# Tariq-Abuhashim/semantic-slam

Measured on AMD Instinct MI355X. Metric: Mvoxels/sec integrated, 512³ grid @ 640×480 depth; achieved HBM GB/s %peak, higher is better.
Workload: dtype f32

## Files before the change

### include/tsdf_hip_diag.h

```cpp
#ifndef TSDF_HIP_DIAG_H
#define TSDF_HIP_DIAG_H

#include "tsdf_hip.h"

#ifdef __cplusplus
extern "C" {
#endif


int tsdf_integrate_sequence_timed(tsdf_volume *vol, const float *depth_dev, const float *cam2world,
                                  int32_t n_frames, float *elapsed_ms);

int tsdf_integrate_frames_timed(tsdf_volume *vol, const float *const *depth_dev, const uint8_t *const *masks_dev,
                                const float *cam2world, int32_t n_frames, float *elapsed_ms);


int tsdf_probe_graph_replay(tsdf_volume *vol, const float *depth_dev, const float *cam2world, int32_t n_frames,
                            int32_t iters, float *ms_launches, float *ms_graph);

int tsdf_probe_stream(tsdf_volume *vol, int32_t non_temporal, int32_t n_iters, float *elapsed_ms);


int tsdf_selftest_fastdiv(int32_t device, uint64_t seed, uint64_t n_samples, float fx, float cx,
                          uint64_t *mismatches, float first_bad[4]);

int tsdf_selftest_fastdiv_band(int32_t device, uint64_t seed, uint64_t n_samples, uint64_t *mismatches,
                               float first_bad[4]);

int tsdf_selftest_round(int32_t device, uint64_t *mismatches, float first_bad[4]);

int tsdf_selftest_tile_tables(int32_t device, const float *depth_dev, const uint8_t *mask_dev, int32_t im_height,
                              int32_t im_width, float max_depth, uint64_t *mismatches);


int32_t tsdf_frames_per_launch(const tsdf_volume *vol);
int tsdf_shortcut_stats(tsdf_volume *vol, int32_t enable, uint64_t counts_out[3]);
int tsdf_brick_list_stats(tsdf_volume *vol, uint64_t counts_out[4]);
int tsdf_classification_info(tsdf_volume *vol, double info_out[2]);

int tsdf_summary_stats(tsdf_volume *vol, uint64_t out[3]);
int tsdf_summary_words(tsdf_volume *vol, uint32_t *out_host, int64_t capacity, int64_t *count);

int tsdf_store_stats(tsdf_volume *vol, int64_t out[9]);

int tsdf_last_cam2base(const tsdf_volume *vol, float out[16]);


int tsdf_set_kernel_variant(tsdf_volume *vol, int32_t variant);

int tsdf_set_brick_shape(tsdf_volume *vol, int32_t quads, int32_t rows, int32_t slices);
int tsdf_brick_shape(const tsdf_volume *vol, int32_t shape_out[3]);
int tsdf_default_brick_shape(const tsdf_config *cfg, int32_t shape_out[3]);

#ifdef __cplusplus
}
#endif
#endif
```

### semantic_slam_amd/capi.py

```python
import ctypes as C
import os

import numpy as np

_PKG = os.path.dirname(os.path.abspath(__file__))
LIB_PATH = os.environ.get("TSDF_HIP_LIB") or os.path.join(_PKG, "libtsdf_hip.so")

ABI_SYMBOLS = [
    "tsdf_config_default", "tsdf_create", "tsdf_destroy", "tsdf_reset", "tsdf_integrate",
    "tsdf_integrate_u16", "tsdf_convert_depth_u16", "tsdf_set_deferral",
    "tsdf_integrate_device", "tsdf_integrate_cam2base", "tsdf_integrate_masked_device",
    "tsdf_integrate_frames_device",
    "tsdf_sync", "tsdf_download", "tsdf_copy_slices", "tsdf_upload", "tsdf_refresh_summary", "tsdf_device_ptrs", "tsdf_slab_voxels", "tsdf_frames_per_launch", "tsdf_shortcut_stats", "tsdf_brick_list_stats", "tsdf_classification_info", "tsdf_store_stats", "tsdf_summary_stats", "tsdf_summary_words",
    "tsdf_get_config", "tsdf_last_cam2base", "tsdf_set_stream", "tsdf_get_stream",
    "tsdf_count_surface", "tsdf_extract_surface", "tsdf_extract_crossings", "tsdf_extract_mesh", "tsdf_save_mesh_ply", "tsdf_save_mesh_welded_ply", "tsdf_save_ply", "tsdf_save_bin", "tsdf_load_bin", "tsdf_save_state", "tsdf_load_state",
    "tsdf_integrate_sequence_timed", "tsdf_integrate_frames_timed", "tsdf_probe_graph_replay", "tsdf_probe_stream", "tsdf_selftest_fastdiv", "tsdf_selftest_fastdiv_band", "tsdf_selftest_round", "tsdf_selftest_tile_tables", "tsdf_set_kernel_variant", "tsdf_set_brick_shape", "tsdf_brick_shape", "tsdf_default_brick_shape", "tsdf_last_error",
    "tsdf_version", "tsdf_multiply_matrix", "tsdf_invert_matrix",
    "tsdf_labels_enable", "tsdf_compose_labels", "tsdf_integrate_labels_device", "tsdf_integrate_frames_labels_device",
    "tsdf_download_labels",
    "tsdf_colour_enable", "tsdf_integrate_colour_device", "tsdf_integrate_rgbd", "tsdf_download_colour",
    "tsdf_raycast_params_default", "tsdf_raycast_device", "tsdf_raycast", "tsdf_batch_raycast_device",
    "tsdf_track_params_default", "tsdf_track", "tsdf_track_system",
    "tsdf_photo_params_default", "tsdf_track_rgbd", "tsdf_track_rgbd_system", "tsdf_render_intensity",
    "tsdf_batch_track", "tsdf_batch_track_system", "tsdf_track_member_systems",
    "tsdf_fuse_params_default", "tsdf_fuse_volume",
    "tsdf_align_params_default", "tsdf_fuse_pose_default", "tsdf_align_volume", "tsdf_align_system", "tsdf_fuse_volume_at",
    "tsdf_fuse_volume_carry", "tsdf_upload_labels", "tsdf_upload_colour",
    "tsdf_extent_params_default", "tsdf_volume_extent", "tsdf_batch_extents", "tsdf_group_extent", "tsdf_extent_combine",
    "tsdf_extent_metric", "tsdf_extent_regrid",
    "tsdf_associate_params_default", "tsdf_associate_count", "tsdf_associate_assign", "tsdf_batch_associate",
    "tsdf_segment_params_default", "tsdf_segmenter_create", "tsdf_segmenter_destroy", "tsdf_segmenter_set_stream",
    "tsdf_segment_depth_device", "tsdf_segment_refine_masks_device", "tsdf_segment_frame",
    "tsdf_object_origin", "tsdf_batch_create", "tsdf_batch_destroy", "tsdf_batch_size", "tsdf_batch_volume",
    "tsdf_batch_integrate_device", "tsdf_batch_sync",
    "tsdf_group_create", "tsdf_group_destroy", "tsdf_group_size", "tsdf_group_voxels", "tsdf_group_volume",
    "tsdf_group_integrate", "tsdf_group_integrate_frames", "tsdf_group_set_deferral", "tsdf_group_sync", "tsdf_group_reset", "tsdf_group_download",
    "tsdf_group_extract_surface", "tsdf_group_extract_crossings", "tsdf_group_extract_mesh",
    "tsdf_group_save_ply", "tsdf_group_save_mesh_ply", "tsdf_group_save_bin",
]
DIAG_SYMBOLS = [
    "tsdf_integrate_sequence_timed", "tsdf_integrate_frames_timed",
    "tsdf_probe_graph_replay", "tsdf_probe_stream",
    "tsdf_selftest_fastdiv", "tsdf_selftest_fastdiv_band", "tsdf_selftest_round", "tsdf_selftest_tile_tables",
    "tsdf_shortcut_stats", "tsdf_brick_list_stats", "tsdf_classification_info", "tsdf_store_stats", "tsdf_summary_stats", "tsdf_summary_words", "tsdf_frames_per_launch", "tsdf_last_cam2base",
    "tsdf_set_kernel_variant", "tsdf_set_brick_shape", "tsdf_brick_shape", "tsdf_default_brick_shape",
]


class TsdfError(RuntimeError):
    pass


SHIPPED_VARIANTS = (0, 1, 3, 7, 8)


def experiments_build():
    return b"+experiments" in load().tsdf_version()


def variants(*wanted):
# ... 147 lines not shown
    L.tsdf_integrate_masked_device.argtypes = [vp, vp, vp, vp]
    L.tsdf_integrate_frames_device.argtypes = [vp, vp, vp, vp, C.c_int32]
    L.tsdf_sync.argtypes = [vp]
    L.tsdf_download.argtypes = [vp, vp, vp]
    L.tsdf_upload.argtypes = [vp, vp, vp]
    L.tsdf_copy_slices.argtypes = [vp, C.c_int32, C.c_int32, vp, vp]
    L.tsdf_refresh_summary.argtypes = [vp]
    L.tsdf_device_ptrs.argtypes = [vp, C.POINTER(vp), C.POINTER(vp)]
    L.tsdf_slab_voxels.argtypes = [vp]
    L.tsdf_slab_voxels.restype = C.c_int64
    L.tsdf_frames_per_launch.argtypes = [vp]
    L.tsdf_frames_per_launch.restype = C.c_int32
    L.tsdf_shortcut_stats.argtypes = [vp, C.c_int32, vp]
    L.tsdf_classification_info.argtypes = [vp, vp]
    L.tsdf_brick_list_stats.argtypes = [vp, vp]
    if hasattr(L, "tsdf_store_stats"):
        L.tsdf_store_stats.argtypes = [vp, i64p]
    if hasattr(L, "tsdf_summary_stats"):
        L.tsdf_summary_stats.argtypes = [vp, vp]
    if hasattr(L, "tsdf_summary_words"):
        L.tsdf_summary_words.argtypes = [vp, vp, C.c_int64, i64p]
    L.tsdf_get_config.argtypes = [vp, C.POINTER(TsdfConfig)]
    L.tsdf_last_cam2base.argtypes = [vp, vp]
    L.tsdf_set_stream.argtypes = [vp, vp]
    L.tsdf_get_stream.argtypes = [vp, C.POINTER(vp)]
    L.tsdf_count_surface.argtypes = [vp, C.c_float, i64p]
    L.tsdf_extract_surface.argtypes = [vp, C.c_float, vp, C.c_int64, i64p]
    L.tsdf_extract_crossings.argtypes = [vp, vp, vp, C.c_float, vp, C.c_int64, i64p]
    L.tsdf_extract_mesh.argtypes = [vp, vp, vp, C.c_float, vp, C.c_int64, i64p]
    L.tsdf_save_mesh_ply.argtypes = [vp, C.c_char_p, C.c_float]
# ... 401 lines not shown
    def shortcut_stats(self, enable=True):
        out = (C.c_uint64 * 3)()
        check(self.lib.tsdf_shortcut_stats(self._h, 1 if enable else 0, out), "tsdf_shortcut_stats")
        return tuple(int(x) for x in out)

    def brick_list_stats(self):
        out = (C.c_uint64 * 4)()
        check(self.lib.tsdf_brick_list_stats(self._h, out), "tsdf_brick_list_stats")
        return tuple(int(x) for x in out)

    def classification_info(self):
        out = (C.c_double * 2)()
        check(self.lib.tsdf_classification_info(self._h, out), "tsdf_classification_info")
        return float(out[0]), int(out[1])

    def store_stats(self):
        out = (C.c_int64 * 9)()
        check(self.lib.tsdf_store_stats(self._h, out), "tsdf_store_stats")
        return {name: tuple(int(x) for x in out[3 * k:3 * k + 3]) for k, name in enumerate(("frames", "masks", "tables"))}

    def summary_stats(self):
        out = (C.c_uint64 * 3)()
        check(self.lib.tsdf_summary_stats(self._h, out), "tsdf_summary_stats")
        return tuple(int(x) for x in out)

    def summary_words(self):
        n = C.c_int64(0)
        check(self.lib.tsdf_summary_words(self._h, None, 0, C.byref(n)), "tsdf_summary_words")
        out = np.zeros(int(n.value), np.uint32)
        if out.size:
# ... 607 lines not shown
```

### semantic_slam_amd/csrc/host_derive.h

```cpp
#pragma once
#include <algorithm>
#include <cmath>
#include <cstddef>
#include <cstdint>

#include "tsdf_hip.h"

namespace tsdf_host {

inline bool brick_shape_ok(const tsdf_config &c, int q, int r, int s)
{
    return c.dim_x % 4 == 0 && q >= 1 && r >= 1 && s >= 1 && q * r * s <= 64 && (c.dim_x / 4) % q == 0 &&
           (long long)s * c.dim_x * c.dim_y < (1ll << 30);
}

inline void choose_brick_default(const tsdf_config &c, int &bq, int &br, int &bs)
{
    bq = 0; br = 0; bs = 1;
    if (c.dim_x % 4 != 0) return;
    const int quads = c.dim_x / 4;
    const int nz = c.z_end - c.z_begin;
    double best = 1e300;
    for (int q = 1; q <= 64 && q <= quads; ++q) {
        if (quads % q) continue;
// ... 132 lines not shown
constexpr int64_t kClassifyMinVoxels = 48000000;
inline bool classify_one_frame(Classify mode, int64_t launch_voxels)
{
    if (mode == Classify::Never) return false;
    return mode == Classify::Always || launch_voxels >= kClassifyMinVoxels;
}

constexpr double kMinClaimFraction = 0.10;
constexpr int kProbeEvery = 8;
inline bool classify_fused(Classify mode, bool claims_known, double claim_fraction, int launches_unclassified)
{
    if (mode != Classify::Adaptive) return mode == Classify::Always;
    return !claims_known || claim_fraction >= kMinClaimFraction || launches_unclassified >= kProbeEvery - 1;
}

constexpr int64_t kWindowBytes = 512ll << 20;

struct SweepWindow { int cache_lo, cache_hi; };

inline SweepWindow sweep_window(int nz, int dim_x, int dim_y, int64_t window_bytes, bool reverse)
{
    const int64_t slice_bytes = 8 * (int64_t)dim_x * dim_y;
    const int w = (int)std::min<int64_t>(nz, window_bytes / slice_bytes);
    return reverse ? SweepWindow{0, w} : SweepWindow{nz - w, nz};
}

inline bool batch_defers(int members, int64_t total_voxels) { return 2 * (int64_t)members < 10 + total_voxels / 1000000; }

constexpr int64_t kBatchMinVoxelsPerMember = 2000000;
inline bool batch_classifies(Classify mode, int members, int64_t launch_voxels)
// ... 45 lines not shown
```

### semantic_slam_amd/csrc/launch_geometry.h

```cpp
#pragma once
#include <algorithm>
#include <cmath>
#include <cstddef>
#include <cstdint>

#include "host_derive.h"

namespace tsdf_host {

enum class ConfigLimit { Ok, GridDims, SlabRange, ImageSize, VoxelAndTrunc, LaunchLimits, SliceVoxels };

constexpr int kMaxDimY = 65535 * 4, kMaxSlices = 65535;
constexpr int64_t kMaxSliceVoxels = ((int64_t)1 << 31) - 1024, kMaxImagePixels = (int64_t)1 << 30;

inline ConfigLimit config_limits_ok(const tsdf_config &c)
{
    if (c.dim_x <= 0 || c.dim_y <= 0 || c.dim_z <= 0) return ConfigLimit::GridDims;
    if (c.z_begin < 0 || c.z_end < c.z_begin || c.z_end > c.dim_z) return ConfigLimit::SlabRange;
    if (c.im_height <= 0 || c.im_width <= 0 || (int64_t)c.im_height * c.im_width > kMaxImagePixels) return ConfigLimit::ImageSize;
    if (!(c.voxel_size > 0.0f) || !(c.trunc_margin > 0.0f)) return ConfigLimit::VoxelAndTrunc;
    if (c.dim_y > kMaxDimY || (c.z_end - c.z_begin) > kMaxSlices) return ConfigLimit::LaunchLimits;
    if ((int64_t)c.dim_x * c.dim_y > kMaxSliceVoxels) return ConfigLimit::SliceVoxels;
    return ConfigLimit::Ok;
}
// ... 57 lines not shown
inline Grid3 grid_quad_rows(const SlabGeometry &g, int rows_per_wg)
{
    return {(unsigned)ceil_div(g.xgroups(4), 64), (unsigned)ceil_div(g.dim_y, rows_per_wg), (unsigned)g.nz};
}
inline Grid3 grid_flat(const SlabGeometry &g) { return {(unsigned)ceil_div(g.chunks_per_slice, 4), 1u, (unsigned)g.nz}; }
inline Grid3 grid_recompute_flags(const SlabGeometry &g) { return grid_flat(g); }

inline int brick_blocks(const SlabGeometry &g) { return ceil_div(g.brick_groups * g.bricks_per_group, 4); }
struct BrickGrid { Grid3 grid; size_t class_elems; };
inline BrickGrid brick_grid(int blocks, int slice_groups)
{
    return {{(unsigned)blocks, 1u, (unsigned)slice_groups}, (size_t)blocks * (size_t)slice_groups * 4};
}
inline BrickGrid brick_grid(const SlabGeometry &g) { return brick_grid(brick_blocks(g), g.nz_groups); }

constexpr size_t kStridePassBlocks = 256 * 8;
inline Grid3 grid_summary_words(const SlabGeometry &g) { return {(unsigned)std::min((g.n_flags + 255) / 256, kStridePassBlocks), 1u, 1u}; }
inline Grid3 grid_fill(const SlabGeometry &g)
{
    return {(unsigned)std::max<size_t>(std::min(((size_t)g.n_vox / 4 + 255) / 256, kStridePassBlocks), 1), 1u, 1u};
}

inline Grid3 grid_tile_strips(int tiles_w, int tiles_h, int tile, int frames)
{
    const int strips = ceil_div(tiles_w, 64 / tile) * tiles_h;
    return {(unsigned)ceil_div(strips, 4), (unsigned)frames, 1u};
}

constexpr int kListBuckets = 64;
constexpr int kSuperBX = 4, kSuperBY = 2, kSuperBZ = 1;
// ... 102 lines not shown
```

### semantic_slam_amd/csrc/tsdf_capi.hip

```cpp
#include "../../include/tsdf_hip.h"
#include "../../include/tsdf_hip_diag.h"

#include <hip/hip_runtime.h>

#include <algorithm>
#include <cmath>
#include <cstdarg>
#include <cstdio>
#include <cstdlib>
#include <cstring>
#include <new>
#include <string>
#include <vector>

#include "pose_math.h"
#include "host_derive.h"
#include "launch_geometry.h"
#include "host_copy.h"
#include "hip_owned.h"
#include "frame_store.h"
#include "tsdf_kernels.hip.h"
#include "tsdf_multiframe.hip.h"
#include "tsdf_labels.hip.h"
#include "tsdf_colour.hip.h"
// ... 102 lines not shown
    DevPtr<unsigned long long> d_claims;
    HostPtr<unsigned long long> h_claims;
    Event claims_done;
    Stream pre_stream, rb_stream;
    int rb_parity = -1;
    Event pre_done[2], list_free[2], seq_ready;
    int list_parity = 0;
    bool list_used[2] = {false, false};
    bool pipeline_ok = false;
    bool claims_pending = false, claims_known = false;
    double claims_total = 0.0;
    double claim_fraction = 0.0;
    int launches_unclassified = 0;
    DevBuf<char> d_scratch;
    DevBuf<uint8_t> d_wg_class;
    DevBuf<char> d_list;
    DevBuf<char> d_track;
    HostPtr<tsdfk::TrackState> h_track;
    DevBuf<char> d_photo;
    HostBuf<char> h_photo;
    DevPtr<unsigned long long> d_fuse;
    HostPtr<unsigned long long> h_fuse;
    Event fuse_src_ready, fuse_done;
    DevPtr<char> d_align;
    HostPtr<tsdfk::TrackState> h_align;
    Event align_src_ready, align_done;
    DevPtr<unsigned long long> d_extent;
    HostPtr<unsigned long long> h_extent;
};

// ... 336 lines not shown
{
    int64_t window = tsdf_host::kWindowBytes;
    bool forward_only = false;
#ifdef TSDF_EXPERIMENTS
    if (const char *e = std::getenv("TSDF_MALL_WINDOW_MB")) window = (int64_t)std::atoi(e) << 20;
    forward_only = std::getenv("TSDF_SWEEP_FORWARD") && std::atoi(std::getenv("TSDF_SWEEP_FORWARD")) != 0;
    p.head_plain_loads = std::getenv("TSDF_HEAD_PLAIN_LOADS") && std::atoi(std::getenv("TSDF_HEAD_PLAIN_LOADS")) != 0;
#endif
    p.sweep_reverse = forward_only ? 0 : v->sweep_parity;
    v->sweep_parity ^= 1;
    const tsdf_host::SweepWindow w = tsdf_host::sweep_window(p.nz, p.dim_x, p.dim_y, window, p.sweep_reverse != 0);
    p.cache_lo = w.cache_lo;
    p.cache_hi = w.cache_hi;
}

int launch_integrate(tsdf_volume *v, const float *depth_dev, const uint8_t *mask_dev,
                     const float *c2b)
{
    const tsdf_host::SlabGeometry &geo = v->geo;
    if (geo.nz == 0) return TSDF_OK;
    std::memcpy(v->last_cam2base, c2b, sizeof v->last_cam2base);
#ifdef TSDF_EXPERIMENTS
    if (geo.quad_rows && (v->variant == 2 || (v->variant >= 16 && !mask_dev) ||
                          (v->variant == 11 && mask_dev && !geo.flat && tiles_fit(geo.tiles_w, geo.tiles_h))))
        return launch_integrate_experiment(v, depth_dev, mask_dev, c2b);
#endif
    const tsdf_host::OneFrame one = tsdf_host::one_frame(geo, variant_of(v->variant), mask_dev != nullptr, tiles_fit(geo.tiles_w, geo.tiles_h));
    if (one.kernel == tsdf_host::OneFrameKernel::Scalar) {
        int rc = summary_before(v, one.keeps);
        if (rc) return rc;
// ... 1 lines not shown
        const dim3 block(64, 4, 1), grid = to_dim3(tsdf_host::grid_scalar_rows(geo));
        if (mask_dev) hipLaunchKernelGGL((tsdfk::integrate_scalar<true>), grid, block, 0, v->stream, p);
        else hipLaunchKernelGGL((tsdfk::integrate_scalar<false>), grid, block, 0, v->stream, p);
        HIP_TRY(hipGetLastError());
        return TSDF_OK;
    }
    if (geo.flat) {
        return launch_multi(v, &depth_dev, mask_dev ? &mask_dev : nullptr, c2b, 1);
    }
    tsdfk::IntegrateParams p = make_params(v, depth_dev, mask_dev, c2b, 4);
    if (one.kernel == tsdf_host::OneFrameKernel::MaskedBricks) return launch_masked_bricks(v, p);
    int rc = summary_before(v, one.keeps);
    if (rc) return rc;
    const dim3 block(64, 4, 1), grid = to_dim3(tsdf_host::grid_quad_rows(geo, 8));
    set_sweep(v, p);
    if (mask_dev) hipLaunchKernelGGL((tsdfk::integrate_tile<2, true>), grid, block, 0, v->stream, p);
    else hipLaunchKernelGGL((tsdfk::integrate_tile<2, false>), grid, block, 0, v->stream, p);
    HIP_TRY(hipGetLastError());
    return TSDF_OK;
}

void compose_cam2base(const tsdf_volume *v, const float *cam2world, float *c2b)
{
    tsdf_host::multiply_matrix(v->base2world_inv, cam2world, c2b);
}

int launch_multi(tsdf_volume *v, const float *const *depth_dev, const uint8_t *const *masks_dev,
                 const float *c2b, int n, const uint16_t *const *label_ims, const float *const *score_ims, hipEvent_t inputs_ready)
{
    const tsdf_config &c = v->cfg;
    const tsdf_host::SlabGeometry &geo = v->geo;
    if (geo.nz == 0 || n == 0) return TSDF_OK;
    {
        int rc = summary_before(v, tsdf_host::Keeps::Bits);
// ... 936 lines not shown
```

### semantic_slam_amd/csrc/tsdf_diag.hip.h

```cpp
#pragma once

namespace {

template <typename Queue>
int time_on_stream(tsdf_volume *v, const char *who, float *elapsed_ms, Queue &&queue)
{
    Event e0, e1;
    HIP_TRY(event_create(e0, hipEventDefault));
    HIP_TRY(event_create(e1, hipEventDefault));
    HIP_TRY(hipEventRecord(e0, v->stream));
    const int rc = queue();
    hipError_t er = hipEventRecord(e1, v->stream);
    hipError_t es = hipEventSynchronize(e1);
    float ms = 0.f;
    hipError_t et = hipEventElapsedTime(&ms, e0, e1);
    if (rc) return rc;
    if (er != hipSuccess || es != hipSuccess || et != hipSuccess)
        return fail(TSDF_ERR_HIP, "%s: event timing failed", who);
    *elapsed_ms = ms;
    return TSDF_OK;
}

int frames_timed(tsdf_volume *v, const float *const *depth_dev, const uint8_t *const *masks_dev,
                 const float *cam2world, int32_t n_frames, float *elapsed_ms, const char *who)
// ... 257 lines not shown
{
    if (!v) return fail(TSDF_ERR_INVALID, "tsdf_shortcut_stats: NULL handle");
    int rc = bind_device(v);
    if (rc) return rc;
    HIP_TRY(hipStreamSynchronize(v->stream));
    if (counts_out) {
        unsigned int h[3] = {0, 0, 0};
        if (v->d_shortcut_stats) HIP_TRY(hipMemcpy(h, v->d_shortcut_stats, sizeof h, hipMemcpyDeviceToHost));
        for (int i = 0; i < 3; ++i) counts_out[i] = h[i];
    }
    if (enable && !v->d_shortcut_stats) HIP_TRY(dev_alloc(v->d_shortcut_stats, 8 * sizeof(unsigned int)));
    if (v->d_shortcut_stats) {
        if (enable) HIP_TRY(hipMemset(v->d_shortcut_stats, 0, 8 * sizeof(unsigned int)));
        else v->d_shortcut_stats.reset();
    }
    return TSDF_OK;
}

int tsdf_brick_list_stats(tsdf_volume *v, uint64_t counts_out[4])
{
    if (!v || !counts_out) return fail(TSDF_ERR_INVALID, "tsdf_brick_list_stats: NULL argument");
    int rc = bind_device(v);
    if (rc) return rc;
    HIP_TRY(hipStreamSynchronize(v->stream));
    unsigned int h[8] = {0, 0, 0, 0, 0, 0, 0, 0};
    if (v->d_shortcut_stats) HIP_TRY(hipMemcpy(h, v->d_shortcut_stats, sizeof h, hipMemcpyDeviceToHost));
    for (int i = 0; i < 4; ++i) counts_out[i] = h[3 + i];
    return TSDF_OK;
}

// ... 59 lines not shown
    std::memcpy(out, v->last_cam2base, sizeof v->last_cam2base);
    return TSDF_OK;
}


int tsdf_set_kernel_variant(tsdf_volume *v, int32_t variant)
{
    if (!v) return fail(TSDF_ERR_INVALID, "tsdf_set_kernel_variant: NULL handle");
    if (!variant_of(variant).known)
        return fail(TSDF_ERR_INVALID, "tsdf_set_kernel_variant: unknown variant %d (this build knows 0, 1, 3, 7, 8%s)", variant,
                    kExperiments ? " and the experiments" : "; the others live in the -DTSDF_EXPERIMENTS build");
    v->variant = variant;
    return TSDF_OK;
}

int tsdf_set_brick_shape(tsdf_volume *v, int32_t quads, int32_t rows, int32_t slices)
{
    if (!v) return fail(TSDF_ERR_INVALID, "tsdf_set_brick_shape: NULL handle");
    if (quads == 0 && rows == 0 && slices == 0) { choose_brick(v); return TSDF_OK; }
    if (!brick_shape_ok(v->cfg, quads, rows, slices))
        return fail(TSDF_ERR_INVALID, "tsdf_set_brick_shape: %d quads x %d rows x %d slices: needs quads * rows * slices <= 64 and "
                    "quads dividing dim_x / 4 = %d", quads, rows, slices, v->cfg.dim_x / 4);
    set_brick(v, quads, rows, slices);
    return TSDF_OK;
}

int tsdf_brick_shape(const tsdf_volume *v, int32_t shape_out[3])
{
    if (!v || !shape_out) return fail(TSDF_ERR_INVALID, "tsdf_brick_shape: NULL argument");
    shape_out[0] = v->geo.brick_q; shape_out[1] = v->geo.brick_q ? v->geo.brick_r : 0; shape_out[2] = v->geo.brick_q ? v->geo.brick_s : 0;
// ... 16 lines not shown
```

### semantic_slam_amd/csrc/tsdf_kernels.hip.h

```cpp
#pragma once
#include <hip/hip_runtime.h>
#include <stdint.h>
#include <type_traits>

#include "host_derive.h"

namespace tsdfk {

struct IntegrateParams {
    const float *depth;
    const uint8_t *mask;
    float *tsdf;
    float *weight;
    float fx, fy, cx, cy;
    float rx0, rx1, rx2;
    float ry0, ry1, ry2;
    float rz0, rz1, rz2;
    float tx, ty, tz;
    float ox, oy, oz;
    float vs, trunc, max_depth;
    int dim_x, dim_y;
    int nz, z_begin;
    int H, W;
    int xgroups;
// ... 159 lines not shown

__device__ __forceinline__ std::true_type weights_nt(std::true_type, uint32_t) { return {}; }
__device__ __forceinline__ bool weights_nt(std::false_type, uint32_t word) { return tsdf_host::word_has_run(word); }
__device__ __forceinline__ bool weights_nt(bool nt, uint32_t word) { return nt || tsdf_host::word_has_run(word); }

__device__ __forceinline__ float gather_f32(const float *__restrict__ base, uint32_t px)
{
    return *reinterpret_cast<const float *>(reinterpret_cast<const char *>(base) + (px << 2));
}

__device__ __forceinline__ int pixel_index24(int iv, int W, int iu)
{
    return (int)(__umul24((unsigned)iv, (unsigned)W) + (unsigned)iu);
}

template <int R, int MASKED>
__device__ __forceinline__ void integrate_tile_body(const IntegrateParams &p, const int bx, const int by, const int lz,
                                                    const bool lnt, const bool snt)
{
    const int gz = p.z_begin + lz;
    const int xg = bx * 64 + threadIdx.x;
    const int gy0 = (by * 4 + threadIdx.y) * R;
    if (xg >= p.xgroups || gy0 >= p.dim_y) return;
    const size_t row0 = ((size_t)lz * p.dim_y + gy0) * (size_t)p.dim_x + (size_t)xg * 4;
    const size_t flag0 = ((size_t)lz * p.dim_y + gy0) * (size_t)p.nseg + bx;

    uint32_t fl[R];
    float4 t4[R], w4[R];
#pragma unroll
    for (int r = 0; r < R; ++r) {
        fl[r] = gy0 + r < p.dim_y ? p.flags[flag0 + (size_t)r * p.nseg] : 0u;
        t4[r] = make_float4(1.f, 1.f, 1.f, 1.f);
        w4[r] = make_float4(0.f, 0.f, 0.f, 0.f);
    }

    float ax[4], ay[4], az[4];
#pragma unroll
    for (int j = 0; j < 4; ++j) {
        float bx = p.ox + (float)(xg * 4 + j) * p.vs;
        float dx = bx - p.tx;
        ax[j] = p.rx0 * dx; ay[j] = p.ry0 * dx; az[j] = p.rz0 * dx;
    }
    const float bz = p.oz + (float)gz * p.vs;
    const float dz = bz - p.tz;
    const float x2 = p.rx2 * dz, y2 = p.ry2 * dz, z2 = p.rz2 * dz;

    float pcz[R][4], dval[R][4];
    bool geo[R][4];
    int pixel[R][4];
#pragma unroll
    for (int r = 0; r < R; ++r) {
        const float dy = (p.oy + (float)(gy0 + r) * p.vs) - p.ty;
        const float z1 = p.rz1 * dy;
#pragma unroll
        for (int j = 0; j < 4; ++j) pcz[r][j] = az[j] + z1 + z2;
    }
    const float cmin = fminf(fminf(pcz[0][0], pcz[0][3]), fminf(pcz[R - 1][0], pcz[R - 1][3]));
    const float cmax = fmaxf(fmaxf(pcz[0][0], pcz[0][3]), fmaxf(pcz[R - 1][0], pcz[R - 1][3]));
    const bool unsafe = !(cmin > p.cz_margin) & !(cmax < -p.cz_margin);
    const bool fast = p.fast_ok != 0 && __ballot(unsafe) == 0ull;
    if (fast) {
        const v2f F = {p.fx, p.fy}, C = {p.cx, p.cy};
        const bool front = cmin > p.cz_margin;
#pragma unroll
        for (int r = 0; r < R; ++r) {
            const bool row_ok = gy0 + r < p.dim_y;
            const float dy = (p.oy + (float)(gy0 + r) * p.vs) - p.ty;
            const v2f XY1 = {p.rx1 * dy, p.ry1 * dy};
            const v2f XY2 = {x2, y2};
#pragma unroll
            for (int j = 0; j < 4; ++j) {
                const v2f A = {ax[j], ay[j]};
                const v2f n = A + XY1 + XY2;
                const float cz = pcz[r][j];
                const v2f uv = F * fast_div2(n, cz) + C;
// ... 25 lines not shown
                pixel[r][j] = ok ? (int)pv * p.W + (int)pu : 0;
            }
        }
    }
#pragma unroll
    for (int r = 0; r < R; ++r) {
#pragma unroll
        for (int j = 0; j < 4; ++j) {
            const uint32_t px = (uint32_t)pixel[r][j];
            float d = gather_f32(p.depth, px);
            if (MASKED == 1) d = d * (p.mask[px] >= 128 ? 1.0f : 0.0f);
            dval[r][j] = d;
        }
    }

    float diff[R][4];
    bool upd[R][4], rowany[R], bandr[R];
    bool any = false, band = false;
#pragma unroll
    for (int r = 0; r < R; ++r) {
        rowany[r] = false;
        bandr[r] = false;
#pragma unroll
        for (int j = 0; j < 4; ++j) {
            const float d = dval[r][j];
            const float df = d - pcz[r][j];
            diff[r][j] = df;
            const bool u = geo[r][j] & !((d <= 0.0f) | (d > p.max_depth)) & !(df <= -p.trunc);
            upd[r][j] = u;
            rowany[r] |= u;
            bandr[r] |= u & !(df >= p.trunc);
        }
        band |= bandr[r];
        any |= rowany[r];
    }
    if (__ballot(any) == 0ull) return;
    if (!any) return;

#pragma unroll
    for (int r = 0; r < R; ++r) fl[r] = __builtin_amdgcn_readfirstlane(fl[r]);
#pragma unroll
    for (int r = 0; r < R; ++r) {
        if (rowany[r]) {
            const float *wp = p.weight + row0 + (size_t)r * p.dim_x, *tp = p.tsdf + row0 + (size_t)r * p.dim_x;
            if (tsdf_host::word_has_run(fl[r])) {
                const float c = (float)tsdf_host::word_run_count(fl[r]);
                w4[r] = make_float4(c, c, c, c);
            } else {
                w4[r] = vol_load_p(lnt, wp);
            }
            if (!(fl[r] & 1u)) t4[r] = vol_load_p(lnt, tp);
        }
// ... 67 lines not shown
            if (rowany[r]) {
                if (word != fl[r]) p.flags[flag0 + (size_t)r * p.nseg] = word;
                if (store_t) vol_store_p(snt_c, p.tsdf + row0 + (size_t)r * p.dim_x, make_float4(tv[0], tv[1], tv[2], tv[3]));
                vol_store_p(weights_nt(snt_c, fl[r]), p.weight + row0 + (size_t)r * p.dim_x, make_float4(wv[0], wv[1], wv[2], wv[3]));
            }
        }
    };
    if constexpr (MASKED == 1) {
        if (snt) store_rows(std::true_type{});
        else store_rows(std::false_type{});
    } else {
        store_rows(snt);
    }
}

template <int R, bool MASKED>
__global__ __launch_bounds__(256) void integrate_tile(IntegrateParams p)
{
    const int lz = p.sweep_reverse ? p.nz - 1 - (int)blockIdx.z : (int)blockIdx.z;
    const bool cached = lz >= p.cache_lo && lz < p.cache_hi;
#ifdef TSDF_EXPERIMENTS
    const bool lnt = !cached && !p.head_plain_loads;
#else
    const bool lnt = !cached;
#endif
    integrate_tile_body<R, MASKED ? 1 : 0>(p, blockIdx.x, blockIdx.y, lz, lnt, !cached);
}

__device__ __forceinline__ uint32_t hash32(uint64_t x)
{
    x ^= x >> 33; x *= 0xff51afd7ed558ccdull; x ^= x >> 33; x *= 0xc4ceb9fe1a85ec53ull; x ^= x >> 33;
    return (uint32_t)x;
}

__global__ __launch_bounds__(256) void selftest_fastdiv(uint64_t seed, uint64_t n_samples, float fx, float cx,
                                                        unsigned long long *mismatch, float *first_bad)
{
    const uint64_t stride = (uint64_t)gridDim.x * blockDim.x;
    for (uint64_t i = (uint64_t)blockIdx.x * blockDim.x + threadIdx.x; i < n_samples; i += stride) {
        const uint32_t h0 = hash32(seed + 3 * i), h1 = hash32(seed + 3 * i + 1), h2 = hash32(seed + 3 * i + 2);
        const uint32_t mode = h2 & 7u;
// ... 195 lines not shown
```

### semantic_slam_amd/csrc/tsdf_multiframe.hip.h

```cpp
#pragma once
#include "launch_geometry.h"
#include "tsdf_kernels.hip.h"

namespace tsdfk {

constexpr int kMaxFramesPerLaunch = 32;
constexpr int kFineTile = 4;
constexpr int kFineLevels = 3;
__host__ __device__ inline size_t fine_table_elems(int fw, int fh) { return (size_t)kFineLevels * kFineLevels * fw * fh; }

struct FramePose {
    const float *depth;
    const uint8_t *mask;
    float rx0, ry0, rx1, ry1, rx2, ry2, rz0, rz1, rz2, tz, tx, ty;
    int fast_ok;
    float cz_margin;
    const uint16_t *label_im;
    const float *score_im;
    const float2 *tiles;
    float cz_short;
    float cz_pad;
};

constexpr int kListBuckets = 64;
// ... 503 lines not shown
    const int id = blockIdx.x * 256 + threadIdx.x;
    if (id >= max_blocks * total_groups * 4) return;
    const int wave = id & 3, wg = (id >> 2) % max_blocks, z = (id >> 2) / max_blocks;
    const int2 m = group_map[z];
    const IntegrateParams p = params[m.x];
    const int brick = wg * 4 + wave;
    const int g = brick / p.bricks_per_group, i = brick - g * p.bricks_per_group;
    int c = 2;
    if (g < p.brick_groups) {
        const int xa = i * p.brick_q * 4, ya = g * p.brick_r;
        const int z0 = m.y * p.brick_s, z1 = min(z0 + p.brick_s - 1, p.nz - 1);
        c = classify_patch(p, class_pose(poses[m.x]), xa, xa + p.brick_q * 4 - 1, ya, min(ya + p.brick_r - 1, p.dim_y - 1), p.z_begin + z0,
                           p.z_begin + z1);
    }
    cls[id] = (uint8_t)c;
}

struct LabelState {
    uint16_t *label;
    float *fp, *bp;
    float prob_thd;
};

struct MultiParamsInline {
    IntegrateParams common;
    FramePose frames[kMaxFramesPerLaunch];
    int n_frames;
    LabelState labels;
    int z_fastest;
#ifdef TSDF_EXPERIMENTS
// ... 609 lines not shown
```

Before: 485,900.

## Pre-classify tile row pairs to skip or shortcut single-frame integration work

Adds a classification pre-pass for single-frame unmasked integration. It builds depth tile tables, then classifies each 256x2 row-pair segment per slice as project, free space or skip. The integrate kernel reads that class and returns early for skip segments, or writes truncated free-space values without projecting. An adaptive host policy enables claims only for large volumes and when the measured share of decided segments is high, and it re-probes periodically through an async counter read-back. The cost is an extra tile-table build and classify launch per frame, plus code-size growth in the kernel.

```diff
diff --git a/include/tsdf_hip_diag.h b/include/tsdf_hip_diag.h
--- a/include/tsdf_hip_diag.h
+++ b/include/tsdf_hip_diag.h
@@ -37,6 +37,7 @@
 int tsdf_shortcut_stats(tsdf_volume *vol, int32_t enable, uint64_t counts_out[3]);
 int tsdf_brick_list_stats(tsdf_volume *vol, uint64_t counts_out[4]);
 int tsdf_classification_info(tsdf_volume *vol, double info_out[2]);
+int tsdf_tile_claim_stats(tsdf_volume *vol, uint64_t counts_out[3]);
 
 int tsdf_summary_stats(tsdf_volume *vol, uint64_t out[3]);
 int tsdf_summary_words(tsdf_volume *vol, uint32_t *out_host, int64_t capacity, int64_t *count);
@@ -48,6 +49,8 @@
 
 int tsdf_set_kernel_variant(tsdf_volume *vol, int32_t variant);
 
+int tsdf_set_tile_claim_min_voxels(tsdf_volume *vol, int64_t min_voxels);
+
 int tsdf_set_brick_shape(tsdf_volume *vol, int32_t quads, int32_t rows, int32_t slices);
 int tsdf_brick_shape(const tsdf_volume *vol, int32_t shape_out[3]);
 int tsdf_default_brick_shape(const tsdf_config *cfg, int32_t shape_out[3]);
diff --git a/semantic_slam_amd/capi.py b/semantic_slam_amd/capi.py
--- a/semantic_slam_amd/capi.py
+++ b/semantic_slam_amd/capi.py
@@ -11,10 +11,10 @@
     "tsdf_integrate_u16", "tsdf_convert_depth_u16", "tsdf_set_deferral",
     "tsdf_integrate_device", "tsdf_integrate_cam2base", "tsdf_integrate_masked_device",
     "tsdf_integrate_frames_device",
-    "tsdf_sync", "tsdf_download", "tsdf_copy_slices", "tsdf_upload", "tsdf_refresh_summary", "tsdf_device_ptrs", "tsdf_slab_voxels", "tsdf_frames_per_launch", "tsdf_shortcut_stats", "tsdf_brick_list_stats", "tsdf_classification_info", "tsdf_store_stats", "tsdf_summary_stats", "tsdf_summary_words",
+    "tsdf_sync", "tsdf_download", "tsdf_copy_slices", "tsdf_upload", "tsdf_refresh_summary", "tsdf_device_ptrs", "tsdf_slab_voxels", "tsdf_frames_per_launch", "tsdf_shortcut_stats", "tsdf_brick_list_stats", "tsdf_classification_info", "tsdf_tile_claim_stats", "tsdf_store_stats", "tsdf_summary_stats", "tsdf_summary_words",
     "tsdf_get_config", "tsdf_last_cam2base", "tsdf_set_stream", "tsdf_get_stream",
     "tsdf_count_surface", "tsdf_extract_surface", "tsdf_extract_crossings", "tsdf_extract_mesh", "tsdf_save_mesh_ply", "tsdf_save_mesh_welded_ply", "tsdf_save_ply", "tsdf_save_bin", "tsdf_load_bin", "tsdf_save_state", "tsdf_load_state",
-    "tsdf_integrate_sequence_timed", "tsdf_integrate_frames_timed", "tsdf_probe_graph_replay", "tsdf_probe_stream", "tsdf_selftest_fastdiv", "tsdf_selftest_fastdiv_band", "tsdf_selftest_round", "tsdf_selftest_tile_tables", "tsdf_set_kernel_variant", "tsdf_set_brick_shape", "tsdf_brick_shape", "tsdf_default_brick_shape", "tsdf_last_error",
+    "tsdf_integrate_sequence_timed", "tsdf_integrate_frames_timed", "tsdf_probe_graph_replay", "tsdf_probe_stream", "tsdf_selftest_fastdiv", "tsdf_selftest_fastdiv_band", "tsdf_selftest_round", "tsdf_selftest_tile_tables", "tsdf_set_kernel_variant", "tsdf_set_tile_claim_min_voxels", "tsdf_set_brick_shape", "tsdf_brick_shape", "tsdf_default_brick_shape", "tsdf_last_error",
     "tsdf_version", "tsdf_multiply_matrix", "tsdf_invert_matrix",
     "tsdf_labels_enable", "tsdf_compose_labels", "tsdf_integrate_labels_device", "tsdf_integrate_frames_labels_device",
     "tsdf_download_labels",
@@ -42,8 +42,8 @@
     "tsdf_integrate_sequence_timed", "tsdf_integrate_frames_timed",
     "tsdf_probe_graph_replay", "tsdf_probe_stream",
     "tsdf_selftest_fastdiv", "tsdf_selftest_fastdiv_band", "tsdf_selftest_round", "tsdf_selftest_tile_tables",
-    "tsdf_shortcut_stats", "tsdf_brick_list_stats", "tsdf_classification_info", "tsdf_store_stats", "tsdf_summary_stats", "tsdf_summary_words", "tsdf_frames_per_launch", "tsdf_last_cam2base",
-    "tsdf_set_kernel_variant", "tsdf_set_brick_shape", "tsdf_brick_shape", "tsdf_default_brick_shape",
+    "tsdf_shortcut_stats", "tsdf_brick_list_stats", "tsdf_classification_info", "tsdf_tile_claim_stats", "tsdf_store_stats", "tsdf_summary_stats", "tsdf_summary_words", "tsdf_frames_per_launch", "tsdf_last_cam2base",
+    "tsdf_set_kernel_variant", "tsdf_set_tile_claim_min_voxels", "tsdf_set_brick_shape", "tsdf_brick_shape", "tsdf_default_brick_shape",
 ]
 
 
@@ -221,6 +221,9 @@
     L.tsdf_shortcut_stats.argtypes = [vp, C.c_int32, vp]
     L.tsdf_classification_info.argtypes = [vp, vp]
     L.tsdf_brick_list_stats.argtypes = [vp, vp]
+    if hasattr(L, "tsdf_tile_claim_stats"):
+        L.tsdf_tile_claim_stats.argtypes = [vp, vp]
+        L.tsdf_set_tile_claim_min_voxels.argtypes = [vp, C.c_int64]
     if hasattr(L, "tsdf_store_stats"):
         L.tsdf_store_stats.argtypes = [vp, i64p]
     if hasattr(L, "tsdf_summary_stats"):
@@ -652,6 +655,14 @@
         check(self.lib.tsdf_classification_info(self._h, out), "tsdf_classification_info")
         return float(out[0]), int(out[1])
 
+    def tile_claim_stats(self):
+        out = (C.c_uint64 * 3)()
+        check(self.lib.tsdf_tile_claim_stats(self._h, out), "tsdf_tile_claim_stats")
+        return tuple(int(x) for x in out)
+
+    def set_tile_claim_min_voxels(self, min_voxels):
+        check(self.lib.tsdf_set_tile_claim_min_voxels(self._h, int(min_voxels)), "tsdf_set_tile_claim_min_voxels")
+
     def store_stats(self):
         out = (C.c_int64 * 9)()
         check(self.lib.tsdf_store_stats(self._h, out), "tsdf_store_stats")
diff --git a/semantic_slam_amd/csrc/host_derive.h b/semantic_slam_amd/csrc/host_derive.h
--- a/semantic_slam_amd/csrc/host_derive.h
+++ b/semantic_slam_amd/csrc/host_derive.h
@@ -170,6 +170,47 @@
     return !claims_known || claim_fraction >= kMinClaimFraction || launches_unclassified >= kProbeEvery - 1;
 }
 
+constexpr int64_t kTileClaimMinVoxels = 40000000;
+constexpr double kTileClaimMinShare = 0.80;
+constexpr int kTileProbeFirst = 8, kTileProbeLast = 256;
+
+struct TileClaimState {
+    bool known = false;
+    double share = 0.0;
+    int unclaimed = 0;
+    int interval = kTileProbeFirst;
+};
+struct TileClaimStep { bool claim; TileClaimState next; };
+
+inline TileClaimStep claim_tile_rows(Classify mode, int64_t launch_voxels, int64_t min_voxels, const TileClaimState &s, bool pending)
+{
+    TileClaimStep r{false, s};
+    if (mode == Classify::Never) return r;
+    if (mode == Classify::Always) { r.claim = true; r.next.unclaimed = 0; return r; }
+    if (launch_voxels < min_voxels) return r;
+    if (s.known ? s.share >= kTileClaimMinShare : !pending) {
+        r.claim = true;
+        r.next.unclaimed = 0;
+        return r;
+    }
+    if (!pending && s.unclaimed >= s.interval - 1) {
+        r.claim = true;
+        r.next.unclaimed = 0;
+        r.next.interval = std::min(2 * s.interval, kTileProbeLast);
+        return r;
+    }
+    r.next.unclaimed = s.unclaimed + 1;
+    return r;
+}
+
+inline TileClaimState tile_claims_read(TileClaimState s, double share)
+{
+    s.known = true;
+    s.share = share;
+    if (share >= kTileClaimMinShare) s.interval = kTileProbeFirst;
+    return s;
+}
+
 constexpr int64_t kWindowBytes = 512ll << 20;
 
 struct SweepWindow { int cache_lo, cache_hi; };
diff --git a/semantic_slam_amd/csrc/launch_geometry.h b/semantic_slam_amd/csrc/launch_geometry.h
--- a/semantic_slam_amd/csrc/launch_geometry.h
+++ b/semantic_slam_amd/csrc/launch_geometry.h
@@ -95,6 +95,15 @@
 }
 inline BrickGrid brick_grid(const SlabGeometry &g) { return brick_grid(brick_blocks(g), g.nz_groups); }
 
+TSDF_HOST_DEVICE inline int tile_row_pairs(int dim_y) { return (dim_y + 1) / 2; }
+TSDF_HOST_DEVICE inline size_t tile_class_index(int lz, int pair, int seg, int pairs, int nseg)
+{
+    return ((size_t)lz * (size_t)pairs + (size_t)pair) * (size_t)nseg + (size_t)seg;
+}
+inline size_t tile_class_elems(const SlabGeometry &g) { return (size_t)g.nz * (size_t)tile_row_pairs(g.dim_y) * (size_t)g.nseg; }
+inline size_t tile_class_alloc(const SlabGeometry &g) { return (tile_class_elems(g) + 3) / 4 * 4; }
+inline Grid3 grid_classify_tile_rows(const SlabGeometry &g) { return {(unsigned)((tile_class_elems(g) + 255) / 256), 1u, 1u}; }
+
 constexpr size_t kStridePassBlocks = 256 * 8;
 inline Grid3 grid_summary_words(const SlabGeometry &g) { return {(unsigned)std::min((g.n_flags + 255) / 256, kStridePassBlocks), 1u, 1u}; }
 inline Grid3 grid_fill(const SlabGeometry &g)
diff --git a/semantic_slam_amd/csrc/tsdf_capi.hip b/semantic_slam_amd/csrc/tsdf_capi.hip
--- a/semantic_slam_amd/csrc/tsdf_capi.hip
+++ b/semantic_slam_amd/csrc/tsdf_capi.hip
@@ -140,6 +140,15 @@
     int launches_unclassified = 0;
     DevBuf<char> d_scratch;
     DevBuf<uint8_t> d_wg_class;
+    DevBuf<uint8_t> d_tile_class;
+    DevPtr<unsigned long long> d_tile_claims;
+    HostPtr<unsigned long long> h_tile_claims;
+    Event tile_claims_done;
+    tsdf_host::TileClaimState tile_policy;
+    bool tile_claims_pending = false;
+    double tile_claims_total = 0.0;
+    bool tile_stats_on = false;
+    int64_t tile_min_voxels = tsdf_host::kTileClaimMinVoxels;
     DevBuf<char> d_list;
     DevBuf<char> d_track;
     HostPtr<tsdfk::TrackState> h_track;
@@ -506,6 +515,101 @@
     p.cache_hi = w.cache_hi;
 }
 
+double tile_claims_read_back(const tsdf_volume *v)
+{
+    double decided = 0.0;
+    for (int s = 0; s < tsdfk::kTileClaimShards; ++s) {
+        const unsigned long long w = v->h_tile_claims[(size_t)s * tsdfk::kTileClaimShardStride];
+        decided += (double)(w >> 32) + (double)(w & 0xffffffffull);
+    }
+    return v->tile_claims_total > 0 ? decided / v->tile_claims_total : 0.0;
+}
+
+int tile_claims_poll(tsdf_volume *v)
+{
+    if (!v->tile_claims_pending) return TSDF_OK;
+    const hipError_t qe = hipEventQuery(v->tile_claims_done);
+    if (qe == hipSuccess) {
+        v->tile_policy = tsdf_host::tile_claims_read(v->tile_policy, tile_claims_read_back(v));
+        v->tile_claims_pending = false;
+    } else if (qe == hipErrorNotReady) {
+        (void)hipGetLastError();
+    } else {
+        v->tile_claims_pending = false;
+        v->tile_policy = tsdf_host::TileClaimState();
+        (void)hipGetLastError();
+        return fail(TSDF_ERR_HIP, "tile claims read-back: hipEventQuery failed: %s", hipGetErrorString(qe));
+    }
+    return TSDF_OK;
+}
+
+int launch_tile_claims(tsdf_volume *v, tsdfk::IntegrateParams &p, bool *claims, bool *counted)
+{
+    *claims = *counted = false;
+    const tsdf_host::SlabGeometry &geo = v->geo;
+    const tsdf_host::Classify mode = variant_of(v->variant).classify;
+    if (mode == tsdf_host::Classify::Never || (mode == tsdf_host::Classify::Adaptive && geo.n_vox < v->tile_min_voxels)) return TSDF_OK;
+    if (!tiles_fit(geo.tiles_w, geo.tiles_h)) return TSDF_OK;
+    hipStreamCaptureStatus cap = hipStreamCaptureStatusNone;
+    HIP_TRY(hipStreamIsCapturing(v->stream, &cap));
+    if (cap != hipStreamCaptureStatusNone) return TSDF_OK;
+    int rc = tile_claims_poll(v);
+    if (rc) return rc;
+    const tsdf_host::TileClaimStep step = tsdf_host::claim_tile_rows(mode, geo.n_vox, v->tile_min_voxels,
+                                                                     v->tile_policy, v->tile_claims_pending);
+    v->tile_policy = step.next;
+    if (!step.claim) return TSDF_OK;
+    if (!v->d_tile_claims) {
+        DevBuf<uint8_t> cls;
+        DevPtr<unsigned long long> dc;
+        HostPtr<unsigned long long> hc;
+        Event ev;
+        hipError_t e = cls.ensure(tsdf_host::tile_class_alloc(geo));
+        if (e == hipSuccess) e = dev_alloc(dc, tsdfk::kTileClaimWords * sizeof(unsigned long long));
+        if (e == hipSuccess) e = hipMemsetAsync(dc, 0, tsdfk::kTileClaimWords * sizeof(unsigned long long), v->stream);
+        if (e == hipSuccess) e = host_alloc(hc, tsdfk::kTileClaimWords * sizeof(unsigned long long), hipHostMallocDefault);
+        if (e == hipSuccess) e = event_create(ev);
+        if (e != hipSuccess) return fail(TSDF_ERR_HIP, "tile claims: %s", hipGetErrorString(e));
+        v->d_tile_class = std::move(cls); v->d_tile_claims = std::move(dc); v->h_tile_claims = std::move(hc); v->tile_claims_done = std::move(ev);
+    }
+    const bool count = !v->tile_claims_pending;
+    constexpr size_t kShardBytes = (size_t)tsdfk::kTileClaimShards * tsdfk::kTileClaimShardStride * sizeof(unsigned long long);
+    StoreSlot table;
+    rc = table.take(v, &v->store->tables, v->stream);
+    if (rc) return rc;
+    if (count) HIP_TRY(hipMemsetAsync(v->d_tile_claims, 0, kShardBytes, v->stream));
+    if (p.tile_inv != 0.0625f) {
+        p.tiles_w = tsdf_host::tiles_along(v->cfg.im_width, 16);
+        p.tiles_h = tsdf_host::tiles_along(v->cfg.im_height, 16);
+        p.tile_inv = 0.0625f;
+    }
+    const float *d = p.depth;
+    rc = build_tile_tables(v->stream, v->cfg, p, &d, nullptr, 1, table.as<float2>());
+    if (rc) return rc;
+    tsdfk::FramePose pose;
+    pose_from_params(pose, p);
+    pose.tiles = table.as<float2>();
+    const size_t n = tsdf_host::tile_class_elems(geo);
+    unsigned long long *const totals = v->tile_stats_on ? v->d_tile_claims + tsdfk::kTileClaimShards * tsdfk::kTileClaimShardStride : nullptr;
+    hipLaunchKernelGGL(tsdfk::classify_tile_rows, to_dim3(tsdf_host::grid_classify_tile_rows(geo)), dim3(256), 0, v->stream, p, pose,
+                       v->d_tile_class.get(), (unsigned long long)n, count ? v->d_tile_claims.get() : nullptr, totals);
+    HIP_TRY(hipGetLastError());
+    p.wg_class = v->d_tile_class;
+    if (count) v->tile_claims_total = (double)n;
+    *claims = true;
+    *counted = count;
+    return table.release();
+}
+
+int tile_claims_send(tsdf_volume *v)
+{
+    constexpr size_t kShardBytes = (size_t)tsdfk::kTileClaimShards * tsdfk::kTileClaimShardStride * sizeof(unsigned long long);
+    HIP_TRY(hipMemcpyAsync(v->h_tile_claims, v->d_tile_claims, kShardBytes, hipMemcpyDeviceToHost, v->stream));
+    HIP_TRY(hipEventRecord(v->tile_claims_done, v->stream));
+    v->tile_claims_pending = true;
+    return TSDF_OK;
+}
+
 int launch_integrate(tsdf_volume *v, const float *depth_dev, const uint8_t *mask_dev,
                      const float *c2b)
 {
@@ -537,10 +641,18 @@
     if (rc) return rc;
     const dim3 block(64, 4, 1), grid = to_dim3(tsdf_host::grid_quad_rows(geo, 8));
     set_sweep(v, p);
-    if (mask_dev) hipLaunchKernelGGL((tsdfk::integrate_tile<2, true>), grid, block, 0, v->stream, p);
+    if (mask_dev) {
+        hipLaunchKernelGGL((tsdfk::integrate_tile<2, true>), grid, block, 0, v->stream, p);
+        HIP_TRY(hipGetLastError());
+        return TSDF_OK;
+    }
+    bool claims = false, counted = false;
+    rc = launch_tile_claims(v, p, &claims, &counted);
+    if (rc) return rc;
+    if (claims) hipLaunchKernelGGL((tsdfk::integrate_tile<2, false, true>), grid, block, 0, v->stream, p);
     else hipLaunchKernelGGL((tsdfk::integrate_tile<2, false>), grid, block, 0, v->stream, p);
     HIP_TRY(hipGetLastError());
-    return TSDF_OK;
+    return counted ? tile_claims_send(v) : TSDF_OK;
 }
 
 void compose_cam2base(const tsdf_volume *v, const float *cam2world, float *c2b)
diff --git a/semantic_slam_amd/csrc/tsdf_diag.hip.h b/semantic_slam_amd/csrc/tsdf_diag.hip.h
--- a/semantic_slam_amd/csrc/tsdf_diag.hip.h
+++ b/semantic_slam_amd/csrc/tsdf_diag.hip.h
@@ -295,6 +295,22 @@
         if (enable) HIP_TRY(hipMemset(v->d_shortcut_stats, 0, 8 * sizeof(unsigned int)));
         else v->d_shortcut_stats.reset();
     }
+    v->tile_stats_on = enable != 0;
+    if (enable && v->d_tile_claims)
+        HIP_TRY(hipMemset(v->d_tile_claims + tsdfk::kTileClaimShards * tsdfk::kTileClaimShardStride, 0, 3 * sizeof(unsigned long long)));
+    return TSDF_OK;
+}
+
+int tsdf_tile_claim_stats(tsdf_volume *v, uint64_t counts_out[3])
+{
+    if (!v || !counts_out) return fail(TSDF_ERR_INVALID, "tsdf_tile_claim_stats: NULL argument");
+    int rc = bind_device(v);
+    if (rc) return rc;
+    HIP_TRY(hipStreamSynchronize(v->stream));
+    unsigned long long h[3] = {0, 0, 0};
+    if (v->d_tile_claims && v->tile_stats_on)
+        HIP_TRY(hipMemcpy(h, v->d_tile_claims + tsdfk::kTileClaimShards * tsdfk::kTileClaimShardStride, sizeof h, hipMemcpyDeviceToHost));
+    for (int i = 0; i < 3; ++i) counts_out[i] = h[i];
     return TSDF_OK;
 }
 
@@ -384,6 +400,13 @@
     return TSDF_OK;
 }
 
+int tsdf_set_tile_claim_min_voxels(tsdf_volume *v, int64_t min_voxels)
+{
+    if (!v) return fail(TSDF_ERR_INVALID, "tsdf_set_tile_claim_min_voxels: NULL handle");
+    v->tile_min_voxels = min_voxels < 0 ? tsdf_host::kTileClaimMinVoxels : min_voxels;
+    return TSDF_OK;
+}
+
 int tsdf_set_brick_shape(tsdf_volume *v, int32_t quads, int32_t rows, int32_t slices)
 {
     if (!v) return fail(TSDF_ERR_INVALID, "tsdf_set_brick_shape: NULL handle");
diff --git a/semantic_slam_amd/csrc/tsdf_kernels.hip.h b/semantic_slam_amd/csrc/tsdf_kernels.hip.h
--- a/semantic_slam_amd/csrc/tsdf_kernels.hip.h
+++ b/semantic_slam_amd/csrc/tsdf_kernels.hip.h
@@ -4,6 +4,7 @@
 #include <type_traits>
 
 #include "host_derive.h"
+#include "launch_geometry.h"
 
 namespace tsdfk {
 
@@ -197,7 +198,7 @@
     return (int)(__umul24((unsigned)iv, (unsigned)W) + (unsigned)iu);
 }
 
-template <int R, int MASKED>
+template <int R, int MASKED, bool CLAIMS = false>
 __device__ __forceinline__ void integrate_tile_body(const IntegrateParams &p, const int bx, const int by, const int lz,
                                                     const bool lnt, const bool snt)
 {
@@ -208,6 +209,17 @@
     const size_t row0 = ((size_t)lz * p.dim_y + gy0) * (size_t)p.dim_x + (size_t)xg * 4;
     const size_t flag0 = ((size_t)lz * p.dim_y + gy0) * (size_t)p.nseg + bx;
 
+    bool claimed_free = false;
+    if constexpr (CLAIMS) {
+        static_assert(MASKED == 0 && R == 2, "claims are built for the unmasked 256 x 2 x 1 wavefront box");
+        const int pair = by * 4 + (int)__builtin_amdgcn_readfirstlane((int)threadIdx.y);
+        const size_t at = tsdf_host::tile_class_index(lz, pair, bx, tsdf_host::tile_row_pairs(p.dim_y), p.nseg);
+        const uint32_t word = reinterpret_cast<const uint32_t *>(p.wg_class)[at >> 2];
+        const uint32_t cls = (word >> (8u * (uint32_t)(at & 3u))) & 0xffu;
+        if (cls == 2u) return;
+        claimed_free = cls == 1u;
+    }
+
     uint32_t fl[R];
     float4 t4[R], w4[R];
 #pragma unroll
@@ -217,6 +229,20 @@
         w4[r] = make_float4(0.f, 0.f, 0.f, 0.f);
     }
 
+    float diff[R][4];
+    bool upd[R][4], rowany[R], bandr[R];
+    bool any = false, band = false;
+    bool fast = false;
+    if (CLAIMS && claimed_free) {
+#pragma unroll
+        for (int r = 0; r < R; ++r) {
+            rowany[r] = gy0 + r < p.dim_y;
+            bandr[r] = false;
+#pragma unroll
+            for (int j = 0; j < 4; ++j) { upd[r][j] = rowany[r]; diff[r][j] = p.trunc; }
+        }
+        any = true;
+    } else {
     float ax[4], ay[4], az[4];
 #pragma unroll
     for (int j = 0; j < 4; ++j) {
@@ -241,7 +267,7 @@
     const float cmin = fminf(fminf(pcz[0][0], pcz[0][3]), fminf(pcz[R - 1][0], pcz[R - 1][3]));
     const float cmax = fmaxf(fmaxf(pcz[0][0], pcz[0][3]), fmaxf(pcz[R - 1][0], pcz[R - 1][3]));
     const bool unsafe = !(cmin > p.cz_margin) & !(cmax < -p.cz_margin);
-    const bool fast = p.fast_ok != 0 && __ballot(unsafe) == 0ull;
+    fast = p.fast_ok != 0 && __ballot(unsafe) == 0ull;
     if (fast) {
         const v2f F = {p.fx, p.fy}, C = {p.cx, p.cy};
         const bool front = cmin > p.cz_margin;
@@ -297,9 +323,6 @@
         }
     }
 
-    float diff[R][4];
-    bool upd[R][4], rowany[R], bandr[R];
-    bool any = false, band = false;
 #pragma unroll
     for (int r = 0; r < R; ++r) {
         rowany[r] = false;
@@ -319,6 +342,7 @@
     }
     if (__ballot(any) == 0ull) return;
     if (!any) return;
+    }
 
 #pragma unroll
     for (int r = 0; r < R; ++r) fl[r] = __builtin_amdgcn_readfirstlane(fl[r]);
@@ -416,7 +440,7 @@
     }
 }
 
-template <int R, bool MASKED>
+template <int R, bool MASKED, bool CLAIMS = false>
 __global__ __launch_bounds__(256) void integrate_tile(IntegrateParams p)
 {
     const int lz = p.sweep_reverse ? p.nz - 1 - (int)blockIdx.z : (int)blockIdx.z;
@@ -426,7 +450,7 @@
 #else
     const bool lnt = !cached;
 #endif
-    integrate_tile_body<R, MASKED ? 1 : 0>(p, blockIdx.x, blockIdx.y, lz, lnt, !cached);
+    integrate_tile_body<R, MASKED ? 1 : 0, CLAIMS>(p, blockIdx.x, blockIdx.y, lz, lnt, !cached);
 }
 
 __device__ __forceinline__ uint32_t hash32(uint64_t x)
diff --git a/semantic_slam_amd/csrc/tsdf_multiframe.hip.h b/semantic_slam_amd/csrc/tsdf_multiframe.hip.h
--- a/semantic_slam_amd/csrc/tsdf_multiframe.hip.h
+++ b/semantic_slam_amd/csrc/tsdf_multiframe.hip.h
@@ -541,6 +541,40 @@
                            p.z_begin + z1);
     }
     cls[id] = (uint8_t)c;
+}
+
+constexpr int kTileClaimShards = 8;
+constexpr int kTileClaimShardStride = 8;
+constexpr int kTileClaimWords = kTileClaimShards * kTileClaimShardStride + 8;
+
+__global__ __launch_bounds__(256) void classify_tile_rows(IntegrateParams p, FramePose pose, uint8_t *cls, unsigned long long n,
+                                                          unsigned long long *counter, unsigned long long *totals)
+{
+    const unsigned long long id = (unsigned long long)blockIdx.x * 256ull + threadIdx.x;
+    const int pairs = tsdf_host::tile_row_pairs(p.dim_y);
+    int c = -1;
+    if (id < n) {
+        const unsigned long long row = id / (unsigned)p.nseg;
+        const int seg = (int)(id - row * (unsigned)p.nseg), lz = (int)(row / (unsigned)pairs), pair = (int)(row - (unsigned long long)lz * (unsigned)pairs);
+        c = classify_patch(p, class_pose(pose), seg * 256, seg * 256 + 255, 2 * pair, min(2 * pair + 1, p.dim_y - 1), p.z_begin + lz);
+        cls[id] = (uint8_t)c;
+    }
+    if (counter == nullptr && totals == nullptr) return;
+    __shared__ unsigned int s_free[4], s_skip[4], s_proj[4];
+    const int wave = threadIdx.x >> 6;
+    const unsigned int nf = (unsigned)__popcll(__ballot(c == 1)), ns = (unsigned)__popcll(__ballot(c == 2)), np = (unsigned)__popcll(__ballot(c == 0));
+    if ((threadIdx.x & 63) == 0) { s_free[wave] = nf; s_skip[wave] = ns; s_proj[wave] = np; }
+    __syncthreads();
+    if (threadIdx.x == 0) {
+        const unsigned long long f = s_free[0] + s_free[1] + s_free[2] + s_free[3], s = s_skip[0] + s_skip[1] + s_skip[2] + s_skip[3];
+        const unsigned long long pr = s_proj[0] + s_proj[1] + s_proj[2] + s_proj[3];
+        if (counter != nullptr && (f | s) != 0ull) atomicAdd(counter + (blockIdx.x % kTileClaimShards) * kTileClaimShardStride, (f << 32) | s);
+        if (totals != nullptr) {
+            if (pr) atomicAdd(totals + 0, pr);
+            if (f) atomicAdd(totals + 1, f);
+            if (s) atomicAdd(totals + 2, s);
+        }
+    }
 }
 
 struct LabelState {
```

After: 488,500 (median of 5 runs). Within noise of the previous version (+0.5%).
